# gplepage/lsqfit

Hardware: AMD Instinct MI355X
Metric: fp64 LM steps/sec at (N_data,N_param)=(65536,4096); chi2 match vs GSL (higher is better)
Workload: dtype f64

## Files before the change

lsqfit_amd/csrc/gemm_tn_f64.hip:

```cpp
#include <cstdlib>

#include "common.h"
#include <type_traits>
#include <vector>
#include "devmath.h"

namespace lsqamd {

#ifdef LSQAMD_SYRK_STAMPS
__device__ unsigned long long *g_syrk_stamps = nullptr;
#endif

typedef double v4d __attribute__((ext_vector_type(4)));
typedef double v2d __attribute__((ext_vector_type(2)));

constexpr int BM = 128, BN = 128, BK = 16;
constexpr int LDT = BM + 16;
constexpr int STAGE = 2 * BK * LDT;
constexpr size_t GEMM_LDS_BYTES = 2 * STAGE * sizeof(double);

struct GemmDev {
  const double *X, *Y;
  double *C;
  int64_t M, N, K, ldx, ldy, ldc;
// ... 22 lines not shown
  v.y = rowptr[i1];
  return v;
}

template <bool VEC>
__global__ __launch_bounds__(256, 2) void gemm_tn_f64_kernel(GemmDev g) {
  extern __shared__ __attribute__((aligned(16))) double smem[];
  const int tid = threadIdx.x;
  const int lane = tid & 63, wave = tid >> 6;
  const int wm = wave >> 1, wn = wave & 1;
  int tm, tn, split;
  if (g.work_map) {
    const int nw = g.n_work, bid = blockIdx.x;
    const int xcd = bid & 7, q = nw >> 3, r = nw & 7;
    const int w = (xcd < r ? xcd * (q + 1) : r * (q + 1) + (xcd - r) * q) + (bid >> 3);
    const int4 e = reinterpret_cast<const int4 *>(g.work_map)[w];
    tm = e.x; tn = e.y; split = e.z;
  } else {
    tm = blockIdx.x / g.tiles_n;
    tn = blockIdx.x % g.tiles_n;
    split = blockIdx.y;
  }
  const int64_t m0 = (int64_t)tm * BM, n0 = (int64_t)tn * BN;
  if (g.upper_only && n0 + BN <= m0) return;

  const int64_t b = blockIdx.z;
  if (g.batch_active && !g.batch_active[b]) return;
  const double *X = g.X + b * g.sx;
  const double *Y = g.Y + b * g.sy;
  double *C = g.C + b * g.sc + (int64_t)split * g.split_stride;

  int64_t kb = (int64_t)split * g.kchunk;
  int64_t ke = kb + g.kchunk < g.K ? kb + g.kchunk : g.K;
  if (g.x_upper_tri) {
    const int64_t lim = m0 + BM;
    if (ke > lim) ke = lim;
  }
  if (g.xy_lower_tri) {
    int64_t lo = m0 > n0 ? m0 : n0;
    lo -= lo % BK;
    if (kb < lo) kb = lo;
  }

  v4d acc[4][4];
#pragma unroll
  for (int i = 0; i < 4; ++i)
#pragma unroll
    for (int j = 0; j < 4; ++j) acc[i][j] = (v4d){0.0, 0.0, 0.0, 0.0};

  const int c2 = (tid & 63) * 2;
  const int rg = tid >> 6;
  const int64_t xc = m0 + c2, yc = n0 + c2;
  const bool x0ok = xc < g.M, x1ok = xc + 1 < g.M;
  const bool y0ok = yc < g.N, y1ok = yc + 1 < g.N;
  const int64_t xi0 = VEC ? (xc < g.ldx - 2 ? xc : g.ldx - 2) : (xc < g.M ? xc : g.M - 1);
  const int64_t xi1 = xc + 1 < g.M ? xc + 1 : g.M - 1;
  const int64_t yi0 = VEC ? (yc < g.ldy - 2 ? yc : g.ldy - 2) : (yc < g.N ? yc : g.N - 1);
  const int64_t yi1 = yc + 1 < g.N ? yc + 1 : g.N - 1;
  v2d xr[4], yr[4];

  auto gload = [&](int64_t k0) {
#pragma unroll
    for (int i = 0; i < 4; ++i) {
      int64_t row = k0 + rg + 4 * i;
      row = row < ke ? row : ke - 1;
      xr[i] = load2<VEC>(X + row * g.ldx, xi0, xi1);
      yr[i] = load2<VEC>(Y + row * g.ldy, yi0, yi1);
    }
  };
  auto sstore = [&](int buf, int64_t k0) {
    double *Xs = smem + buf * STAGE;
    double *Ys = Xs + BK * LDT;
#pragma unroll
    for (int i = 0; i < 4; ++i) {
      const int row = rg + 4 * i;
      const bool rok = k0 + row < ke;
      v2d xv, yv;
      xv.x = (rok && x0ok) ? xr[i].x : 0.0;
      xv.y = (rok && x1ok) ? xr[i].y : 0.0;
      yv.x = (rok && y0ok) ? yr[i].x : 0.0;
      yv.y = (rok && y1ok) ? yr[i].y : 0.0;
      *reinterpret_cast<v2d *>(Xs + row * LDT + c2) = xv;
      *reinterpret_cast<v2d *>(Ys + row * LDT + c2) = yv;
    }
  };

  const int fr = lane & 15, fq = lane >> 4;
  if (kb < ke) {
    gload(kb);
    sstore(0, kb);
  }
  __syncthreads();
  int cur = 0;
  for (int64_t k0 = kb; k0 < ke; k0 += BK) {
    const bool more = k0 + BK < ke;
    if (more) gload(k0 + BK);
    const double *Xs = smem + cur * STAGE;
    const double *Ys = Xs + BK * LDT;
#pragma unroll
    for (int kk = 0; kk < BK / 4; ++kk) {
      const int kr = kk * 4 + fq;
      double a[4], bb[4];
#pragma unroll
      for (int i = 0; i < 4; ++i) a[i] = Xs[kr * LDT + wm * 64 + i * 16 + fr];
#pragma unroll
      for (int j = 0; j < 4; ++j) bb[j] = Ys[kr * LDT + wn * 64 + j * 16 + fr];
#pragma unroll
      for (int i = 0; i < 4; ++i)
#pragma unroll
        for (int j = 0; j < 4; ++j)
          acc[i][j] = __builtin_amdgcn_mfma_f64_16x16x4f64(a[i], bb[j], acc[i][j], 0, 0, 0);
    }
    if (more) sstore(cur ^ 1, k0 + BK);
    __syncthreads();
    cur ^= 1;
  }

  const double alpha = g.alpha;
  const double beta = g.splits > 1 ? 0.0 : g.beta;
#pragma unroll
  for (int i = 0; i < 4; ++i) {
    double cv[4][4];
    if (beta != 0.0) {
#pragma unroll
      for (int j = 0; j < 4; ++j)
#pragma unroll
        for (int r = 0; r < 4; ++r) {
          const int64_t col = n0 + wn * 64 + j * 16 + fr;
          const int64_t row = m0 + wm * 64 + i * 16 + fq + 4 * r;
          const bool ok = col < g.N && row < g.M;
          cv[j][r] = C[(ok ? row : 0) * g.ldc + (ok ? col : 0)];
        }
    }
#pragma unroll
    for (int j = 0; j < 4; ++j) {
      const int64_t col = n0 + wn * 64 + j * 16 + fr;
      if (col >= g.N) continue;
#pragma unroll
      for (int r = 0; r < 4; ++r) {
        const int64_t row = m0 + wm * 64 + i * 16 + fq + 4 * r;
        if (row >= g.M) continue;
        double v = alpha * acc[i][j][r];
        if (beta != 0.0) v += beta * cv[j][r];
        C[row * g.ldc + col] = v;
      }
    }
  }
}

template <bool XTRI, bool WORKMAP, bool CS = false, bool SIGNAL = false>
__global__ __launch_bounds__(256, 2) void gemm_tn_f64_interior_kernel(GemmDev g) {
  extern __shared__ __attribute__((aligned(16))) double smem[];
  const int tid = threadIdx.x;
  const int lane = tid & 63, wave = tid >> 6;
  const int wm = wave >> 1, wn = wave & 1;
  int tm, tn, split;
  int sig_group = 0;
#ifdef LSQAMD_SYRK_STAMPS
  const unsigned long long stamp0 = __builtin_amdgcn_s_memrealtime();
  int stamp_w = -1;
#endif
  if (WORKMAP) {
    const int nw = g.n_work, bid = blockIdx.x;
    const int xcd = bid & 7, q = nw >> 3, r = nw & 7;
    const int w = (xcd < r ? xcd * (q + 1) : r * (q + 1) + (xcd - r) * q) + (bid >> 3);
#ifdef LSQAMD_SYRK_STAMPS
    stamp_w = w;
#endif
    const int4 e = reinterpret_cast<const int4 *>(g.work_map)[w];
    tm = e.x; tn = e.y; split = e.z;
    if (SIGNAL) sig_group = e.w;
  } else if (XTRI && g.xcd_groups) {
    const int L = blockIdx.x, xcd = L & 7, sl = L >> 3;
    const int gidx = xcd + 8 * (sl / g.tiles_n);
    tn = sl % g.tiles_n;
    tm = gidx % g.xcd_groups;
    split = gidx / g.xcd_groups;
  } else {
    tm = blockIdx.x / g.tiles_n;
    tn = blockIdx.x % g.tiles_n;
    split = blockIdx.y;
  }
  const int tm_other = (XTRI && g.pair_rows) ? g.tiles_m - 1 - tm : tm;
  const int npass = tm_other != tm ? 2 : 1;
  for (int pass = 0; pass < npass; ++pass) {
  if (pass >= 1) {
    tm = tm_other;
    __syncthreads();
  }
  const int64_t m0 = (int64_t)tm * BM, n0 = (int64_t)tn * BN;
  if (g.upper_only && n0 + BN <= m0) return;
  const int64_t b = blockIdx.z;
  if (g.batch_active && !g.batch_active[b]) return;
  double *C = g.C + b * g.sc + (int64_t)split * g.split_stride;
  int64_t kb = (int64_t)split * g.kchunk;
  int64_t ke = kb + g.kchunk < g.K ? kb + g.kchunk : g.K;
  if (g.x_upper_tri) {
    const int64_t lim = m0 + BM;
    if (ke > lim) ke = lim;
  }
  if (g.xy_lower_tri) {
    int64_t lo = m0 > n0 ? m0 : n0;
    lo -= lo % BK;
    if (kb < lo) kb = lo;
  }
  if (XTRI && g.tri_halves) {
    const int64_t lim = m0 + BM, h = (lim >> 1) & ~(int64_t)(BK - 1);
    kb = split ? h : 0;
    ke = split ? lim : h;
  }

  v4d acc[4][4];
#pragma unroll
  for (int i = 0; i < 4; ++i)
#pragma unroll
    for (int j = 0; j < 4; ++j) acc[i][j] = (v4d){0.0, 0.0, 0.0, 0.0};

  const bool diag = WORKMAP && !XTRI && g.syrk_diag && tm == tn;
  const int arow0 = diag ? (wave == 2 ? 32 : (wave == 3 ? 64 : 0)) : wm * 64;
  const int bcol0 = diag ? (wave == 0 ? 0 : 64) : wn * 64;

  typedef __attribute__((address_space(3))) void lds_void;
  typedef const __attribute__((address_space(1))) void glb_void;
  const double *xp = g.X + b * g.sx + (kb + wave) * g.ldx + m0 + 2 * lane;
  const double *yp = g.Y + b * g.sy + (kb + wave) * g.ldy + n0 + 2 * lane;
  const int64_t xstep = 4 * g.ldx, ystep = 4 * g.ldy;
  const char *fp = reinterpret_cast<const char *>(g.X + b * g.sx + (kb + (lane >> 1)) * g.ldx + g.colsum_rcol) + 4 * (lane & 1);
  const int64_t fstep = (int64_t)BK * g.ldx * (int64_t)sizeof(double);
  double cs = 0.0, cs2 = 0.0;

  auto stage = [&](int buf) {
    double *Xs = smem + buf * STAGE + wave * LDT;
    double *Ys = Xs + BK * LDT;
    if (diag) {
#pragma unroll
      for (int i = 0; i < 4; ++i)
        __builtin_amdgcn_global_load_lds((glb_void *)(xp + i * xstep), (lds_void *)(Xs + 4 * i * LDT), 16, 0, 0);
      if (CS && wave == 1) {
        if (lane < 32)
          __builtin_amdgcn_global_load_lds((glb_void *)fp, (lds_void *)(smem + buf * STAGE + BK * LDT), 4, 0, 0);
        fp += fstep;
      }
    } else {
#pragma unroll
      for (int i = 0; i < 4; ++i) {
        __builtin_amdgcn_global_load_lds((glb_void *)(xp + i * xstep), (lds_void *)(Xs + 4 * i * LDT), 16, 0, 0);
        __builtin_amdgcn_global_load_lds((glb_void *)(yp + i * ystep), (lds_void *)(Ys + 4 * i * LDT), 16, 0, 0);
      }
    }
    xp += 4 * xstep;
    yp += 4 * ystep;
  };

  const bool fuse = XTRI && g.colsum_out != nullptr;
  double wreg = 0.0;
  if (fuse && tid < BM) wreg = (g.C + b * g.sc)[(m0 + tid) * g.ldc + g.colsum_rcol];
  const int fr = lane & 15, fq = lane >> 4;
  if (kb < ke) stage(0);
  __syncthreads();
  auto kloop = [&](auto role_tag) {
    constexpr int ROLE = decltype(role_tag)::value;
    int cur = 0;
    for (int64_t k0 = kb; k0 < ke; k0 += BK) {
      if (k0 + BK < ke) stage(cur ^ 1);
      const double *Xs = smem + cur * STAGE;
      const double *Ys = ROLE == 0 ? Xs + BK * LDT : Xs;
#pragma unroll
      for (int kk = 0; kk < BK / 4; ++kk) {
        const int kr = kk * 4 + fq;
        double a[4], bb[4];
#pragma unroll
        for (int i = 0; i < (ROLE == 2 ? 2 : 4); ++i)
          a[i] = Xs[kr * LDT + (XTRI ? (2 * i + wm) * 16 : arow0 + i * 16) + fr];
#pragma unroll
        for (int j = 0; j < 4; ++j) bb[j] = Ys[kr * LDT + bcol0 + j * 16 + fr];
#pragma unroll
        for (int i = 0; i < (ROLE == 2 ? 2 : 4); ++i) {
          if (XTRI && k0 + kk * 4 > m0 + (2 * i + wm) * 16 + 15) continue;
#pragma unroll
          for (int j = (ROLE == 1 ? i : 0); j < 4; ++j)
            acc[i][j] = __builtin_amdgcn_mfma_f64_16x16x4f64(a[i], bb[j], acc[i][j], 0, 0, 0);
        }
      }
      if (CS && ROLE != 0) {
        const double *Fs = Xs + BK * LDT + 8 * (tid >> 7);
        const double *Xc = Xs + 8 * (tid >> 7) * LDT + (tid & 127);
#pragma unroll
        for (int r = 0; r < 8; ++r) {
          const double fv = Fs[r];
          cs = fma(Xc[r * LDT], fv, cs);
          cs2 = fma(fv, fv, cs2);
        }
      }
      __syncthreads();
      cur ^= 1;
    }
  };
  if (WORKMAP && !XTRI && diag) {
    if (wave == 0 || wave == 3) kloop(std::integral_constant<int, 1>{});
    else kloop(std::integral_constant<int, 2>{});
    const double alpha = g.alpha;
    const bool tri = wave == 0 || wave == 3;
#pragma unroll
    for (int i = 0; i < 4; ++i) {
      if (!tri && i >= 2) break;
#pragma unroll
      for (int j = 0; j < 4; ++j) {
        if (tri && j < i) continue;
        const int64_t col = n0 + bcol0 + j * 16 + fr;
#pragma unroll
        for (int r = 0; r < 4; ++r) {
          const int64_t row = m0 + arow0 + i * 16 + fq + 4 * r;
          const double v = alpha * acc[i][j][r];
          C[row * g.ldc + col] = v;
          if (!(tri && i == j)) C[col * g.ldc + row] = v;
        }
      }
    }
    if (CS) {
      smem[tid] = cs;
      if ((tid & 127) == 0) smem[256 + (tid >> 7)] = cs2;
      __syncthreads();
      double *out = g.colsum_out + (b * g.splits + split) * g.colsum_ld;
      if (tid < BM) out[m0 + tid] = smem[tid] + smem[tid + 128];
      if (tm == 0 && tid == 0) out[g.colsum_rcol] = smem[256] + smem[257];
    }
    continue;
  }
  kloop(std::integral_constant<int, 0>{});

  const double alpha = g.alpha;
  const double beta = g.splits > 1 ? 0.0 : g.beta;
  double *wcol = smem;
  double *red = smem + 128;
  if (fuse) {
    if (tid < BM) wcol[tid] = wreg;
    __syncthreads();
  }
  double sj[4] = {0.0, 0.0, 0.0, 0.0};
#pragma unroll
  for (int i = 0; i < 4; ++i) {
    const int rloc = (XTRI ? (2 * i + wm) * 16 : wm * 64 + i * 16) + fq;
    const int64_t rbase = m0 + rloc;
    double cv[4][4];
    if (beta != 0.0) {
#pragma unroll
      for (int j = 0; j < 4; ++j)
#pragma unroll
        for (int r = 0; r < 4; ++r)
          cv[j][r] = C[(rbase + 4 * r) * g.ldc + n0 + wn * 64 + j * 16 + fr];
    }
#pragma unroll
    for (int r = 0; r < 4; ++r) {
      const double w = fuse ? wcol[rloc + 4 * r] : 0.0;
#pragma unroll
      for (int j = 0; j < 4; ++j) {
        double v = alpha * acc[i][j][r];
        if (beta != 0.0) v += beta * cv[j][r];
        C[(rbase + 4 * r) * g.ldc + n0 + wn * 64 + j * 16 + fr] = v;
        if (XTRI) sj[j] += v * w;
      }
    }
  }
  if (fuse) {
#pragma unroll
    for (int j = 0; j < 4; ++j) {
      sj[j] += __shfl_xor(sj[j], 16, 64);
      sj[j] += __shfl_xor(sj[j], 32, 64);
    }
    if (fq == 0) {
#pragma unroll
      for (int j = 0; j < 4; ++j) red[wave * 64 + j * 16 + fr] = sj[j];
    }
    __syncthreads();
    if (wm == 0 && fq == 0) {
      double *out = g.colsum_out + (b * g.tiles_m + tm) * g.colsum_ld + n0 + wn * 64;
#pragma unroll
      for (int j = 0; j < 4; ++j) out[j * 16 + fr] = red[wave * 64 + j * 16 + fr] + red[(wave + 2) * 64 + j * 16 + fr];
    }
  }
  }
  if (SIGNAL && WORKMAP && sig_group > 0 && g.done_ctr) {
    asm volatile("s_waitcnt vmcnt(0)" ::: "memory");
    __syncthreads();
    if (tid == 0) {
      __builtin_amdgcn_fence(__ATOMIC_RELEASE, "agent");
      asm volatile("s_waitcnt vmcnt(0)" ::: "memory");
      __hip_atomic_fetch_add(g.done_ctr + (sig_group - 1), 1, __ATOMIC_RELAXED, __HIP_MEMORY_SCOPE_AGENT);
    }
  }
#ifdef LSQAMD_SYRK_STAMPS
  if (WORKMAP && g_syrk_stamps && tid == 0) {
    __builtin_amdgcn_s_waitcnt(0);
    unsigned long long *o = g_syrk_stamps + 5 * (size_t)blockIdx.x;
    o[0] = stamp0;
    o[1] = __builtin_amdgcn_s_memrealtime();
    o[2] = __builtin_amdgcn_s_getreg((3 << 11) | 20);
    o[3] = __builtin_amdgcn_s_getreg((31 << 11) | 4);
    o[4] = (unsigned long long)stamp_w;
  }
#endif
}

constexpr int TS = 64;
constexpr int LDS_S = TS + 16;
constexpr int STAGE_S = 2 * BK * LDS_S;
constexpr size_t GEMM_LDS_BYTES_S = 2 * STAGE_S * sizeof(double);

template <bool VEC>
__global__ __launch_bounds__(256, 4) void gemm_tn_f64_small_kernel(GemmDev g) {
  extern __shared__ __attribute__((aligned(16))) double smem[];
  const int tid = threadIdx.x;
  const int lane = tid & 63, wave = tid >> 6;
  const int wm = wave >> 1, wn = wave & 1;
  const int tm = blockIdx.x / g.tiles_n, tn = blockIdx.x % g.tiles_n;
  const int split = blockIdx.y;
  const int64_t m0 = (int64_t)tm * TS, n0 = (int64_t)tn * TS;
  if (g.upper_only && n0 + TS <= m0) return;
  const int64_t b = blockIdx.z;
  if (g.batch_active && !g.batch_active[b]) return;
  const double *X = g.X + b * g.sx;
  const double *Y = g.Y + b * g.sy;
  double *C = g.C + b * g.sc + (int64_t)split * g.split_stride;
  int64_t kb = (int64_t)split * g.kchunk;
  int64_t ke = kb + g.kchunk < g.K ? kb + g.kchunk : g.K;
  if (g.x_upper_tri) {
    const int64_t lim = m0 + TS;
    if (ke > lim) ke = lim;
  }
  if (g.xy_lower_tri) {
    int64_t lo = m0 > n0 ? m0 : n0;
    lo -= lo % BK;
    if (kb < lo) kb = lo;
  }
  v4d acc[2][2];
#pragma unroll
  for (int i = 0; i < 2; ++i)
#pragma unroll
    for (int j = 0; j < 2; ++j) acc[i][j] = (v4d){0.0, 0.0, 0.0, 0.0};

  const int c2 = (tid & 31) * 2;
  const int rg = tid >> 5;
  const int64_t xc = m0 + c2, yc = n0 + c2;
  const bool x0ok = xc < g.M, x1ok = xc + 1 < g.M;
  const bool y0ok = yc < g.N, y1ok = yc + 1 < g.N;
  const int64_t xi0 = VEC ? (xc < g.ldx - 2 ? xc : g.ldx - 2) : (xc < g.M ? xc : g.M - 1);
  const int64_t xi1 = xc + 1 < g.M ? xc + 1 : g.M - 1;
  const int64_t yi0 = VEC ? (yc < g.ldy - 2 ? yc : g.ldy - 2) : (yc < g.N ? yc : g.N - 1);
// ... 427 lines not shown
      }
    }
    hipLaunchKernelGGL((gemm_tn_f64_interior_kernel<true, false>), grid, dim3(256), GEMM_LDS_BYTES, st, g);
  }
  else if (interior && a.work_map && a.colsum_out) {
    if (!g.syrk_diag || !a.upper_only) return hipErrorInvalidValue;
    if (g.done_ctr) hipLaunchKernelGGL((gemm_tn_f64_interior_kernel<false, true, true, true>), grid, dim3(256), GEMM_LDS_BYTES, st, g);
    else hipLaunchKernelGGL((gemm_tn_f64_interior_kernel<false, true, true>), grid, dim3(256), GEMM_LDS_BYTES, st, g);
  }
  else if (interior && a.work_map && g.done_ctr)
    hipLaunchKernelGGL((gemm_tn_f64_interior_kernel<false, true, false, true>), grid, dim3(256), GEMM_LDS_BYTES, st, g);
  else if (interior && a.work_map)
    hipLaunchKernelGGL((gemm_tn_f64_interior_kernel<false, true>), grid, dim3(256), GEMM_LDS_BYTES, st, g);
  else if (interior)
    hipLaunchKernelGGL((gemm_tn_f64_interior_kernel<false, false>), grid, dim3(256), GEMM_LDS_BYTES, st, g);
  else if (g.vec_x && g.vec_y)
    hipLaunchKernelGGL(gemm_tn_f64_kernel<true>, grid, dim3(256), GEMM_LDS_BYTES, st, g);
  else
    hipLaunchKernelGGL(gemm_tn_f64_kernel<false>, grid, dim3(256), GEMM_LDS_BYTES, st, g);
  return hipGetLastError();
}

int64_t syrk_work_count(int64_t P, int32_t splits) {
  const int64_t T = (P + BM - 1) / BM;
  return T * (T + 1) / 2 * (splits < 1 ? 1 : splits);
}

void syrk_work_fill(int64_t P, int32_t splits, int32_t *out) { (void)syrk_work_fill_rows(P, splits, 0, (int)((P + BM - 1) / BM), out); }

int64_t syrk_work_fill_rows(int64_t P, int32_t splits, int row0, int row1, int32_t *out) {
  const int T = (int)((P + BM - 1) / BM), PS = 8;
  const int NP = (T + PS - 1) / PS;
  if (row0 < 0) row0 = 0;
  if (row1 > T) row1 = T;
  int64_t o = 0;
  for (int s = 0; s < (splits < 1 ? 1 : splits); ++s)
    for (int pi = 0; pi < NP; ++pi)
      for (int pj = pi; pj < NP; ++pj)
        for (int tm = pi * PS; tm < (pi + 1) * PS && tm < T; ++tm) {
          if (tm < row0 || tm >= row1) continue;
          for (int tn = pj * PS; tn < (pj + 1) * PS && tn < T; ++tn) {
            if (tn < tm) continue;
            out[o++] = tm; out[o++] = tn; out[o++] = s; out[o++] = 0;
          }
        }
  const int64_t nw = o / 4, q = nw / 8, r = nw % 8;
  std::vector<int32_t> tmp;
  for (int xcd = 0; xcd < 8; ++xcd) {
    const int64_t b = xcd < r ? xcd * (q + 1) : r * (q + 1) + (xcd - r) * q, n = q + (xcd < r ? 1 : 0);
    tmp.assign(out + 4 * b, out + 4 * (b + n));
    int64_t w = b;
    for (int keep = 0; keep < 2; ++keep)
      for (int64_t e = 0; e < n; ++e)
        if ((tmp[4 * e] == tmp[4 * e + 1]) == (keep == 1)) {
          for (int c = 0; c < 4; ++c) out[4 * w + c] = tmp[4 * e + c];
          ++w;
        }
  }
  return nw;
}

void syrk_work_fill_grouped(int64_t P, int32_t splits, int G, const int32_t *rows, int32_t *out, int32_t *count) {
  const int64_t nw = syrk_work_count(P, splits), q = nw / 8, r = nw % 8;
  std::vector<std::vector<int32_t>> lists((size_t)G);
  for (int g = 0; g < G; ++g) {
    lists[(size_t)g].resize(4 * (size_t)nw);
    const int T = (int)((P + BM - 1) / BM), PS = 8, NP = (T + PS - 1) / PS;
    int64_t o = 0;
    int32_t *L = lists[(size_t)g].data();
    for (int s = 0; s < (splits < 1 ? 1 : splits); ++s)
      for (int pi = 0; pi < NP; ++pi)
        for (int pj = pi; pj < NP; ++pj)
          for (int tm = pi * PS; tm < (pi + 1) * PS && tm < T; ++tm) {
            if (tm < rows[g] || tm >= rows[g + 1]) continue;
            for (int tn = pj * PS; tn < (pj + 1) * PS && tn < T; ++tn) {
              if (tn < tm) continue;
              L[o++] = tm; L[o++] = tn; L[o++] = s; L[o++] = g + 1;
            }
          }
    lists[(size_t)g].resize((size_t)o);
    count[g] = (int32_t)(o / 4);
  }
  std::vector<int64_t> cap(8), pos((size_t)G, 0);
  for (int x = 0; x < 8; ++x) cap[(size_t)x] = q + (x < r ? 1 : 0);
  std::vector<std::vector<int64_t>> c((size_t)G, std::vector<int64_t>(8, 0));
  for (int g = 0; g < G; ++g) {
    if (g == G - 1) {
      for (int x = 0; x < 8; ++x) c[(size_t)g][(size_t)x] = cap[(size_t)x];
      break;
    }
    int64_t left = count[g];
    for (int x = 0; x < 8; ++x) {
      int64_t v = count[g] / 8;
      if (v > cap[(size_t)x]) v = cap[(size_t)x];
      c[(size_t)g][(size_t)x] = v;
      cap[(size_t)x] -= v;
      left -= v;
    }
    while (left > 0) {
      int best = 0;
      for (int x = 1; x < 8; ++x)
        if (cap[(size_t)x] > cap[(size_t)best]) best = x;
      c[(size_t)g][(size_t)best]++;
      cap[(size_t)best]--;
      --left;
    }
  }
  int64_t w = 0;
  for (int x = 0; x < 8; ++x)
    for (int g = 0; g < G; ++g) {
      const int32_t *L = lists[(size_t)g].data() + 4 * pos[(size_t)g];
      const int64_t n = c[(size_t)g][(size_t)x];
      for (int keep = 0; keep < 2; ++keep)
        for (int64_t e = 0; e < n; ++e)
          if ((L[4 * e] == L[4 * e + 1]) == (keep == 1)) {
            for (int k = 0; k < 4; ++k) out[4 * w + k] = L[4 * e + k];
            ++w;
          }
      pos[(size_t)g] += n;
    }
}

__global__ __launch_bounds__(64) void wait_counter_kernel(const int32_t *ctr, int32_t expect, int32_t *timed_out) {
  if (threadIdx.x != 0) return;
  const unsigned long long t0 = __builtin_amdgcn_s_memrealtime();
  while (__hip_atomic_load(ctr, __ATOMIC_RELAXED, __HIP_MEMORY_SCOPE_AGENT) < expect) {
    __builtin_amdgcn_s_sleep(64);
    if (__builtin_amdgcn_s_memrealtime() - t0 > 400000000ull) {
      __hip_atomic_store(timed_out, 1, __ATOMIC_RELAXED, __HIP_MEMORY_SCOPE_AGENT);
      break;
    }
  }
}

hipError_t launch_wait_counter(hipStream_t st, const int32_t *ctr, int32_t expect, int32_t *timed_out) {
  hipLaunchKernelGGL(wait_counter_kernel, dim3(1), dim3(64), 0, st, ctr, expect, timed_out);
  return hipGetLastError();
}

template <int MODEL, int NT, bool FAR>
__global__ __launch_bounds__(256, 2) void whiten_synth_kernel(WhitenSynth a, int tiles_m, int tiles_n, int pair_rows) {
  extern __shared__ __attribute__((aligned(16))) double smem[];
  if (a.trig_far && (a.trig_far[0] != 0) != FAR) return;
  const int tid = threadIdx.x;
  const int lane = tid & 63, wave = __builtin_amdgcn_readfirstlane(tid >> 6);
  const int wm = wave >> 1, wn = wave & 1;
  const int tm_first = blockIdx.x / tiles_n, tn = blockIdx.x % tiles_n;
  const int npass = (pair_rows && tiles_m - 1 - tm_first != tm_first) ? 2 : 1;
  for (int pass = 0; pass < npass; ++pass) {
  if (pass == 1) __syncthreads();
  const int tm = pass == 0 ? tm_first : tiles_m - 1 - tm_first;
  const int64_t b = blockIdx.z;
  const int64_t m0 = (int64_t)tm * BM;
  const int64_t ke = m0 + BM;
  const double *Xb = a.Wt + b * a.B * a.B;
  const double *xrow = a.x + b * a.B;
  double *C = a.J + b * a.B * a.ld;
  constexpr int NJ = NT / 16;
  constexpr int SR = 256 / NT, NS = BK / SR;
  const int sc = tid % NT, srow = tid / NT;
  const double amp = a.p[(int64_t)tn * NT + sc], frq = a.p[a.K + (int64_t)tn * NT + sc];

  v4d acc[4][NJ];
#pragma unroll
  for (int i = 0; i < 4; ++i)
#pragma unroll
    for (int j = 0; j < NJ; ++j) acc[i][j] = (v4d){0.0, 0.0, 0.0, 0.0};
  typedef __attribute__((address_space(3))) void lds_void;
  typedef const __attribute__((address_space(1))) void glb_void;
  const double *xp = Xb + (int64_t)wave * a.B + m0 + 2 * lane;
  const int64_t xstep = 4 * a.B;
  double *xring = smem + 2 * STAGE;
  auto xdma = [&](int64_t sidx) {
    if (wave == 0) {
      int64_t e = sidx * BK + (lane >> 1);
      if (e > a.B - 1) e = a.B - 1;
      const char *src = reinterpret_cast<const char *>(xrow + e) + 4 * (lane & 1);
      __builtin_amdgcn_global_load_lds((glb_void *)src, (lds_void *)(xring + (sidx % 3) * 32), 4, 0, 0);
    }
  };
  int64_t ssyn = 0;
  auto stage_dma = [&](int buf) {
    double *Xs = smem + buf * STAGE + wave * LDT;
#pragma unroll
    for (int i = 0; i < 4; ++i)
      __builtin_amdgcn_global_load_lds((glb_void *)(xp + i * xstep), (lds_void *)(Xs + 4 * i * LDT), 16, 0, 0);
    xp += 4 * xstep;
  };
  auto stage_synth = [&](int buf) {
    double xs4[NS];
    const double *xq = xring + (ssyn % 3) * 32 + srow;
#pragma unroll
    for (int i = 0; i < NS; ++i) xs4[i] = xq[SR * i];
    double *Ys = smem + buf * STAGE + BK * LDT;
#pragma unroll
    for (int i = 0; i < NS; ++i) {
      const int row = srow + SR * i;
      const double xv = xs4[i];
      double t, dq;
      if (MODEL == LSQAMD_MODEL_COSMIX) {
        double sn, cs;
        sincos_moderate<FAR>(frq * xv, &sn, &cs);
        t = cs;
        dq = -amp * xv * sn;
      } else {
        const double e = exp(-frq * xv);
        t = e;
        dq = -amp * xv * e;
      }
      Ys[row * LDT + sc] = t;
      Ys[row * LDT + NT + sc] = dq;
    }
    ++ssyn;
  };
  const double wreg = (tid < BM) ? C[(m0 + tid) * a.ld + 2 * a.K] : 0.0;
  const int fr = lane & 15, fq = lane >> 4;
  xdma(0);
  xdma(1);
  stage_dma(0);
  __syncthreads();
  stage_synth(0);
  __syncthreads();
  int cur = 0;
  for (int64_t k0 = 0; k0 < ke; k0 += BK) {
    if (k0 + BK < ke) {
      if (k0 + 2 * BK < ke) xdma(k0 / BK + 2);
      stage_dma(cur ^ 1);
      stage_synth(cur ^ 1);
    }
    const double *Xs = smem + cur * STAGE;
    const double *Ys = Xs + BK * LDT;
#pragma unroll
    for (int kk = 0; kk < BK / 4; ++kk) {
      const int kr = kk * 4 + fq;
      double av[4], bb[NJ];
#pragma unroll
      for (int i = 0; i < 4; ++i) av[i] = Xs[kr * LDT + (2 * i + wm) * 16 + fr];
#pragma unroll
      for (int j = 0; j < NJ; ++j) bb[j] = Ys[kr * LDT + wn * NT + j * 16 + fr];
#pragma unroll
      for (int i = 0; i < 4; ++i) {
        if (k0 + kk * 4 > m0 + (2 * i + wm) * 16 + 15) continue;
#pragma unroll
        for (int j = 0; j < NJ; ++j)
          acc[i][j] = __builtin_amdgcn_mfma_f64_16x16x4f64(av[i], bb[j], acc[i][j], 0, 0, 0);
      }
    }
    __syncthreads();
    cur ^= 1;
  }
  double *wcol = smem, *red = smem + 128;
  if (tid < BM) wcol[tid] = wreg;
  __syncthreads();
  const int64_t cbase = (wn ? a.K : 0) + (int64_t)tn * NT;
  double sj[NJ];
#pragma unroll
  for (int j = 0; j < NJ; ++j) sj[j] = 0.0;
#pragma unroll
  for (int i = 0; i < 4; ++i) {
    const int rloc = (2 * i + wm) * 16 + fq;
#pragma unroll
    for (int r = 0; r < 4; ++r) {
      const double w = wcol[rloc + 4 * r];
#pragma unroll
      for (int j = 0; j < NJ; ++j) {
        const double v = acc[i][j][r];
        C[(m0 + rloc + 4 * r) * a.ld + cbase + j * 16 + fr] = v;
        sj[j] += v * w;
      }
    }
  }
#pragma unroll
  for (int j = 0; j < NJ; ++j) {
    sj[j] += __shfl_xor(sj[j], 16, 64);
    sj[j] += __shfl_xor(sj[j], 32, 64);
  }
  if (fq == 0) {
#pragma unroll
    for (int j = 0; j < NJ; ++j) red[wave * 64 + j * 16 + fr] = sj[j];
  }
  __syncthreads();
  if (wm == 0 && fq == 0) {
    double *out = a.colsum_out + (b * tiles_m + tm) * (2 * a.K) + cbase;
#pragma unroll
    for (int j = 0; j < NJ; ++j) out[j * 16 + fr] = red[wave * 64 + j * 16 + fr] + red[(wave + 2) * 64 + j * 16 + fr];
  }
  }
}


bool whiten_synth_eligible(int32_t model, int64_t B, int64_t P) {
  const char *e = getenv("LSQAMD_FUSED_JACOBIAN");
  const bool off = e && e[0] == '0', always = e && e[0] == '2';
  return !off && (model == LSQAMD_MODEL_COSMIX || model == LSQAMD_MODEL_MULTIEXP) && B >= BM && B % BM == 0 &&
         (B < 8 * BM || always) && P % 128 == 0 && P >= 128;
}

constexpr size_t SYNTH_LDS_BYTES = GEMM_LDS_BYTES + 3 * 32 * sizeof(double);

template <int MODEL, int NT, bool FAR>
static hipError_t launch_whiten_synth_one(hipStream_t st, const WhitenSynth &a, dim3 grid, int tiles_m, int tiles_n, int pair) {
  static PerDeviceOnce attr;
  const hipError_t ea = attr.run([] {
    return hipFuncSetAttribute(reinterpret_cast<const void *>(whiten_synth_kernel<MODEL, NT, FAR>),
                               hipFuncAttributeMaxDynamicSharedMemorySize, (int)SYNTH_LDS_BYTES);
  });
  if (ea != hipSuccess) return ea;
  hipLaunchKernelGGL((whiten_synth_kernel<MODEL, NT, FAR>), grid, dim3(256), SYNTH_LDS_BYTES, st, a, tiles_m, tiles_n, pair);
  return hipGetLastError();
}

template <int MODEL, int NT>
static hipError_t launch_whiten_synth_nt(hipStream_t st, const WhitenSynth &a, dim3 grid, int tiles_m, int tiles_n, int pair) {
  if (MODEL == LSQAMD_MODEL_COSMIX && a.trig_far) {
    hipError_t e = launch_whiten_synth_one<MODEL, NT, false>(st, a, grid, tiles_m, tiles_n, pair);
    if (e != hipSuccess) return e;
  }
  return launch_whiten_synth_one<MODEL, NT, true>(st, a, grid, tiles_m, tiles_n, pair);
}

hipError_t launch_whiten_synth(hipStream_t st, const WhitenSynth &a0) {
  WhitenSynth a = a0;
  if (a.model != LSQAMD_MODEL_COSMIX) a.trig_far = nullptr;
  const int tiles_m = (int)(a.B / BM);
  const int pair = tiles_m >= 4 ? 1 : 0;
  const int64_t rows = pair ? (tiles_m + 1) / 2 : tiles_m;
  static const int64_t narrow_below = [] { const char *e = getenv("LSQAMD_SYNTH_NARROW"); return e ? atoll(e) : (int64_t)400; }();
  const bool narrow = rows * (a.K / 64) * a.nb < narrow_below && a.K % 32 == 0;
  const int tiles_n = (int)(a.K / (narrow ? 32 : 64));
  dim3 grid((unsigned)(rows * tiles_n), 1, (unsigned)a.nb);
  if (a.model == LSQAMD_MODEL_COSMIX)
    return narrow ? launch_whiten_synth_nt<LSQAMD_MODEL_COSMIX, 32>(st, a, grid, tiles_m, tiles_n, pair)
                  : launch_whiten_synth_nt<LSQAMD_MODEL_COSMIX, 64>(st, a, grid, tiles_m, tiles_n, pair);
  return narrow ? launch_whiten_synth_nt<LSQAMD_MODEL_MULTIEXP, 32>(st, a, grid, tiles_m, tiles_n, pair)
                : launch_whiten_synth_nt<LSQAMD_MODEL_MULTIEXP, 64>(st, a, grid, tiles_m, tiles_n, pair);
}

}

#ifdef LSQAMD_SYRK_STAMPS
extern "C" int lsqamd_debug_set_syrk_stamps(void *dev_ptr) try {
  return (int)hipMemcpyToSymbol(HIP_SYMBOL(lsqamd::g_syrk_stamps), &dev_ptr, sizeof(void *));
} LSQAMD_ABI_CATCH(return lsqamd::abi_exception(nullptr);)
#endif
```

Before: 50.03.

## Split k-loop into full and triangular phases with compile-time buffer indices

Restructures the GEMM-TN interior and whiten-synth k-loops. Each loop is unrolled by two with constexpr double-buffer indices, and full stages are separated from the diagonal triangular stages, so the per-MFMA triangle check disappears from the bulk of the loop. Wave and work-map indices are made scalar with readfirstlane, and LDS pointers and a lane offset are precomputed to cut VALU address arithmetic. The cost is more code and higher register pressure, and the new stage counting adds risk of off-by-one errors at tile boundaries.

```diff
diff --git a/lsqfit_amd/csrc/gemm_tn_f64.hip b/lsqfit_amd/csrc/gemm_tn_f64.hip
--- a/lsqfit_amd/csrc/gemm_tn_f64.hip
+++ b/lsqfit_amd/csrc/gemm_tn_f64.hip
@@ -198,7 +198,7 @@
 __global__ __launch_bounds__(256, 2) void gemm_tn_f64_interior_kernel(GemmDev g) {
   extern __shared__ __attribute__((aligned(16))) double smem[];
   const int tid = threadIdx.x;
-  const int lane = tid & 63, wave = tid >> 6;
+  const int lane = tid & 63, wave = __builtin_amdgcn_readfirstlane(tid >> 6);
   const int wm = wave >> 1, wn = wave & 1;
   int tm, tn, split;
   int sig_group = 0;
@@ -214,8 +214,10 @@
     stamp_w = w;
 #endif
     const int4 e = reinterpret_cast<const int4 *>(g.work_map)[w];
-    tm = e.x; tn = e.y; split = e.z;
-    if (SIGNAL) sig_group = e.w;
+    tm = __builtin_amdgcn_readfirstlane(e.x);
+    tn = __builtin_amdgcn_readfirstlane(e.y);
+    split = __builtin_amdgcn_readfirstlane(e.z);
+    if (SIGNAL) sig_group = __builtin_amdgcn_readfirstlane(e.w);
   } else if (XTRI && g.xcd_groups) {
     const int L = blockIdx.x, xcd = L & 7, sl = L >> 3;
     const int gidx = xcd + 8 * (sl / g.tiles_n);
@@ -268,20 +270,24 @@
 
   typedef __attribute__((address_space(3))) void lds_void;
   typedef const __attribute__((address_space(1))) void glb_void;
-  const double *xp = g.X + b * g.sx + (kb + wave) * g.ldx + m0 + 2 * lane;
-  const double *yp = g.Y + b * g.sy + (kb + wave) * g.ldy + n0 + 2 * lane;
-  const int64_t xstep = 4 * g.ldx, ystep = 4 * g.ldy;
+  const char *xb = reinterpret_cast<const char *>(g.X + b * g.sx + (kb + wave) * g.ldx + m0);
+  const char *yb = reinterpret_cast<const char *>(g.Y + b * g.sy + (kb + wave) * g.ldy + n0);
+  const int64_t xstep = 4 * g.ldx * (int64_t)sizeof(double), ystep = 4 * g.ldy * (int64_t)sizeof(double);
+  uint32_t lane_off = 16u * (uint32_t)lane;
+  const int nst = kb < ke ? (int)((ke - kb + BK - 1) >> 4) : 0;
   const char *fp = reinterpret_cast<const char *>(g.X + b * g.sx + (kb + (lane >> 1)) * g.ldx + g.colsum_rcol) + 4 * (lane & 1);
   const int64_t fstep = (int64_t)BK * g.ldx * (int64_t)sizeof(double);
   double cs = 0.0, cs2 = 0.0;
 
-  auto stage = [&](int buf) {
+  auto stage = [&](auto buf_tag) {
+    constexpr int buf = decltype(buf_tag)::value;
+    asm volatile("" : "+v"(lane_off));
     double *Xs = smem + buf * STAGE + wave * LDT;
     double *Ys = Xs + BK * LDT;
     if (diag) {
 #pragma unroll
       for (int i = 0; i < 4; ++i)
-        __builtin_amdgcn_global_load_lds((glb_void *)(xp + i * xstep), (lds_void *)(Xs + 4 * i * LDT), 16, 0, 0);
+        __builtin_amdgcn_global_load_lds((glb_void *)(xb + i * xstep + lane_off), (lds_void *)(Xs + 4 * i * LDT), 16, 0, 0);
       if (CS && wave == 1) {
         if (lane < 32)
           __builtin_amdgcn_global_load_lds((glb_void *)fp, (lds_void *)(smem + buf * STAGE + BK * LDT), 4, 0, 0);
@@ -290,42 +296,69 @@
     } else {
 #pragma unroll
       for (int i = 0; i < 4; ++i) {
-        __builtin_amdgcn_global_load_lds((glb_void *)(xp + i * xstep), (lds_void *)(Xs + 4 * i * LDT), 16, 0, 0);
-        __builtin_amdgcn_global_load_lds((glb_void *)(yp + i * ystep), (lds_void *)(Ys + 4 * i * LDT), 16, 0, 0);
-      }
-    }
-    xp += 4 * xstep;
-    yp += 4 * ystep;
+        __builtin_amdgcn_global_load_lds((glb_void *)(xb + i * xstep + lane_off), (lds_void *)(Xs + 4 * i * LDT), 16, 0, 0);
+        __builtin_amdgcn_global_load_lds((glb_void *)(yb + i * ystep + lane_off), (lds_void *)(Ys + 4 * i * LDT), 16, 0, 0);
+      }
+    }
+    xb += 4 * xstep;
+    yb += 4 * ystep;
   };
 
   const bool fuse = XTRI && g.colsum_out != nullptr;
   double wreg = 0.0;
   if (fuse && tid < BM) wreg = (g.C + b * g.sc)[(m0 + tid) * g.ldc + g.colsum_rcol];
   const int fr = lane & 15, fq = lane >> 4;
-  if (kb < ke) stage(0);
+  if (nst > 0) stage(std::integral_constant<int, 0>{});
   __syncthreads();
   auto kloop = [&](auto role_tag) {
     constexpr int ROLE = decltype(role_tag)::value;
-    int cur = 0;
-    for (int64_t k0 = kb; k0 < ke; k0 += BK) {
-      if (k0 + BK < ke) stage(cur ^ 1);
+    typedef const __attribute__((address_space(3))) double lds_cdouble;
+    lds_cdouble *ap[2][BK / 4], *bp[2][BK / 4];
+#pragma unroll
+    for (int c = 0; c < 2; ++c)
+#pragma unroll
+      for (int kk = 0; kk < BK / 4; ++kk) {
+        const double *Xk = smem + c * STAGE + (kk * 4 + fq) * LDT + fr;
+        ap[c][kk] = (lds_cdouble *)(Xk + (XTRI ? wm * 16 : arow0));
+        bp[c][kk] = (lds_cdouble *)(Xk + (ROLE == 0 ? BK * LDT : 0) + bcol0);
+        asm volatile("" : "+v"(ap[c][kk]), "+v"(bp[c][kk]));
+      }
+    auto body = [&](auto cur_tag, auto tri_tag, const int ts, const bool more) {
+      constexpr int cur = decltype(cur_tag)::value;
+      constexpr bool TRI = XTRI && decltype(tri_tag)::value != 0;
+      if (more) stage(std::integral_constant<int, cur ^ 1>{});
       const double *Xs = smem + cur * STAGE;
-      const double *Ys = ROLE == 0 ? Xs + BK * LDT : Xs;
-#pragma unroll
-      for (int kk = 0; kk < BK / 4; ++kk) {
-        const int kr = kk * 4 + fq;
-        double a[4], bb[4];
-#pragma unroll
-        for (int i = 0; i < (ROLE == 2 ? 2 : 4); ++i)
-          a[i] = Xs[kr * LDT + (XTRI ? (2 * i + wm) * 16 : arow0 + i * 16) + fr];
-#pragma unroll
-        for (int j = 0; j < 4; ++j) bb[j] = Ys[kr * LDT + bcol0 + j * 16 + fr];
-#pragma unroll
-        for (int i = 0; i < (ROLE == 2 ? 2 : 4); ++i) {
-          if (XTRI && k0 + kk * 4 > m0 + (2 * i + wm) * 16 + 15) continue;
-#pragma unroll
-          for (int j = (ROLE == 1 ? i : 0); j < 4; ++j)
-            acc[i][j] = __builtin_amdgcn_mfma_f64_16x16x4f64(a[i], bb[j], acc[i][j], 0, 0, 0);
+      if (TRI) {
+        double bb[BK / 4][4];
+#pragma unroll
+        for (int kk = 0; kk < BK / 4; ++kk)
+#pragma unroll
+          for (int j = 0; j < 4; ++j) bb[kk][j] = bp[cur][kk][j * 16];
+#pragma unroll
+        for (int i = 0; i < 4; ++i) {
+          if (2 * i + wm < ts) continue;
+          double a[BK / 4];
+#pragma unroll
+          for (int kk = 0; kk < BK / 4; ++kk) a[kk] = ap[cur][kk][2 * i * 16];
+#pragma unroll
+          for (int kk = 0; kk < BK / 4; ++kk)
+#pragma unroll
+            for (int j = 0; j < 4; ++j)
+              acc[i][j] = __builtin_amdgcn_mfma_f64_16x16x4f64(a[kk], bb[kk][j], acc[i][j], 0, 0, 0);
+        }
+      } else {
+#pragma unroll
+        for (int kk = 0; kk < BK / 4; ++kk) {
+          double a[4], bb[4];
+#pragma unroll
+          for (int i = 0; i < (ROLE == 2 ? 2 : 4); ++i) a[i] = ap[cur][kk][(XTRI ? 2 * i : i) * 16];
+#pragma unroll
+          for (int j = 0; j < 4; ++j) bb[j] = bp[cur][kk][j * 16];
+#pragma unroll
+          for (int i = 0; i < (ROLE == 2 ? 2 : 4); ++i)
+#pragma unroll
+            for (int j = (ROLE == 1 ? i : 0); j < 4; ++j)
+              acc[i][j] = __builtin_amdgcn_mfma_f64_16x16x4f64(a[i], bb[j], acc[i][j], 0, 0, 0);
         }
       }
       if (CS && ROLE != 0) {
@@ -339,7 +372,32 @@
         }
       }
       __syncthreads();
-      cur ^= 1;
+    };
+    using c0_tag = std::integral_constant<int, 0>;
+    using c1_tag = std::integral_constant<int, 1>;
+    int nfull = nst;
+    if (XTRI) {
+      const int64_t below = kb < m0 ? (m0 - kb) >> 4 : 0;
+      nfull = below < nst ? (int)below : nst;
+    }
+    int s = 0;
+    for (; s + 1 < nfull; s += 2) {
+      body(c0_tag{}, c0_tag{}, 0, true);
+      body(c1_tag{}, c0_tag{}, 0, s + 2 < nst);
+    }
+    if (s < nfull) body(c0_tag{}, c0_tag{}, 0, s + 1 < nst);
+    if (XTRI && nfull < nst) {
+      const int t1 = (int)((kb + (int64_t)nst * BK - m0) >> 4);
+      int t = t1 - (nst - nfull);
+      if (nfull & 1) {
+        body(c1_tag{}, c1_tag{}, t, t + 1 < t1);
+        ++t;
+      }
+      for (; t + 1 < t1; t += 2) {
+        body(c0_tag{}, c1_tag{}, t, true);
+        body(c1_tag{}, c1_tag{}, t + 1, t + 2 < t1);
+      }
+      if (t < t1) body(c0_tag{}, c1_tag{}, t, false);
     }
   };
   if (WORKMAP && !XTRI && diag) {
@@ -1073,7 +1131,6 @@
   const int tm = pass == 0 ? tm_first : tiles_m - 1 - tm_first;
   const int64_t b = blockIdx.z;
   const int64_t m0 = (int64_t)tm * BM;
-  const int64_t ke = m0 + BM;
   const double *Xb = a.Wt + b * a.B * a.B;
   const double *xrow = a.x + b * a.B;
   double *C = a.J + b * a.B * a.ld;
@@ -1089,26 +1146,30 @@
     for (int j = 0; j < NJ; ++j) acc[i][j] = (v4d){0.0, 0.0, 0.0, 0.0};
   typedef __attribute__((address_space(3))) void lds_void;
   typedef const __attribute__((address_space(1))) void glb_void;
-  const double *xp = Xb + (int64_t)wave * a.B + m0 + 2 * lane;
-  const int64_t xstep = 4 * a.B;
+  const char *xb = reinterpret_cast<const char *>(Xb + (int64_t)wave * a.B + m0);
+  const int64_t xstep = 4 * a.B * (int64_t)sizeof(double);
+  uint32_t lane_off = 16u * (uint32_t)lane;
   double *xring = smem + 2 * STAGE;
-  auto xdma = [&](int64_t sidx) {
+  auto xdma = [&](int sidx) {
     if (wave == 0) {
-      int64_t e = sidx * BK + (lane >> 1);
+      int64_t e = (int64_t)sidx * BK + (lane >> 1);
       if (e > a.B - 1) e = a.B - 1;
       const char *src = reinterpret_cast<const char *>(xrow + e) + 4 * (lane & 1);
       __builtin_amdgcn_global_load_lds((glb_void *)src, (lds_void *)(xring + (sidx % 3) * 32), 4, 0, 0);
     }
   };
-  int64_t ssyn = 0;
-  auto stage_dma = [&](int buf) {
+  int ssyn = 0;
+  auto stage_dma = [&](auto buf_tag) {
+    constexpr int buf = decltype(buf_tag)::value;
+    asm volatile("" : "+v"(lane_off));
     double *Xs = smem + buf * STAGE + wave * LDT;
 #pragma unroll
     for (int i = 0; i < 4; ++i)
-      __builtin_amdgcn_global_load_lds((glb_void *)(xp + i * xstep), (lds_void *)(Xs + 4 * i * LDT), 16, 0, 0);
-    xp += 4 * xstep;
+      __builtin_amdgcn_global_load_lds((glb_void *)(xb + i * xstep + lane_off), (lds_void *)(Xs + 4 * i * LDT), 16, 0, 0);
+    xb += 4 * xstep;
   };
-  auto stage_synth = [&](int buf) {
+  auto stage_synth = [&](auto buf_tag) {
+    constexpr int buf = decltype(buf_tag)::value;
     double xs4[NS];
     const double *xq = xring + (ssyn % 3) * 32 + srow;
 #pragma unroll
@@ -1136,19 +1197,25 @@
   };
   const double wreg = (tid < BM) ? C[(m0 + tid) * a.ld + 2 * a.K] : 0.0;
   const int fr = lane & 15, fq = lane >> 4;
+  using c0_tag = std::integral_constant<int, 0>;
+  using c1_tag = std::integral_constant<int, 1>;
   xdma(0);
   xdma(1);
-  stage_dma(0);
+  stage_dma(c0_tag{});
   __syncthreads();
-  stage_synth(0);
+  stage_synth(c0_tag{});
   __syncthreads();
-  int cur = 0;
-  for (int64_t k0 = 0; k0 < ke; k0 += BK) {
-    if (k0 + BK < ke) {
-      if (k0 + 2 * BK < ke) xdma(k0 / BK + 2);
-      stage_dma(cur ^ 1);
-      stage_synth(cur ^ 1);
-    }
+  const int nst = 8 * (tm + 1);
+  auto next = [&](auto cur_tag, const int sidx) {
+    constexpr int cur = decltype(cur_tag)::value;
+    if (sidx + 1 < nst) {
+      if (sidx + 2 < nst) xdma(sidx + 2);
+      stage_dma(std::integral_constant<int, cur ^ 1>{});
+      stage_synth(std::integral_constant<int, cur ^ 1>{});
+    }
+  };
+  auto mfmas_full = [&](auto cur_tag) {
+    constexpr int cur = decltype(cur_tag)::value;
     const double *Xs = smem + cur * STAGE;
     const double *Ys = Xs + BK * LDT;
 #pragma unroll
@@ -1160,15 +1227,50 @@
 #pragma unroll
       for (int j = 0; j < NJ; ++j) bb[j] = Ys[kr * LDT + wn * NT + j * 16 + fr];
 #pragma unroll
-      for (int i = 0; i < 4; ++i) {
-        if (k0 + kk * 4 > m0 + (2 * i + wm) * 16 + 15) continue;
+      for (int i = 0; i < 4; ++i)
 #pragma unroll
         for (int j = 0; j < NJ; ++j)
           acc[i][j] = __builtin_amdgcn_mfma_f64_16x16x4f64(av[i], bb[j], acc[i][j], 0, 0, 0);
-      }
-    }
+    }
+  };
+  auto mfmas_tri = [&](auto cur_tag, const int ts) {
+    constexpr int cur = decltype(cur_tag)::value;
+    const double *Xs = smem + cur * STAGE;
+    const double *Ys = Xs + BK * LDT;
+    double bb[BK / 4][NJ];
+#pragma unroll
+    for (int kk = 0; kk < BK / 4; ++kk)
+#pragma unroll
+      for (int j = 0; j < NJ; ++j) bb[kk][j] = Ys[(kk * 4 + fq) * LDT + wn * NT + j * 16 + fr];
+#pragma unroll
+    for (int i = 0; i < 4; ++i) {
+      if (2 * i + wm < ts) continue;
+      double av[BK / 4];
+#pragma unroll
+      for (int kk = 0; kk < BK / 4; ++kk) av[kk] = Xs[(kk * 4 + fq) * LDT + (2 * i + wm) * 16 + fr];
+#pragma unroll
+      for (int kk = 0; kk < BK / 4; ++kk)
+#pragma unroll
+        for (int j = 0; j < NJ; ++j)
+          acc[i][j] = __builtin_amdgcn_mfma_f64_16x16x4f64(av[kk], bb[kk][j], acc[i][j], 0, 0, 0);
+    }
+  };
+  const int nfull = 8 * tm;
+  for (int s = 0; s < nfull; s += 2) {
+    next(c0_tag{}, s);
+    mfmas_full(c0_tag{});
     __syncthreads();
-    cur ^= 1;
+    next(c1_tag{}, s + 1);
+    mfmas_full(c1_tag{});
+    __syncthreads();
+  }
+  for (int t = 0; t < 8; t += 2) {
+    next(c0_tag{}, nfull + t);
+    mfmas_tri(c0_tag{}, t);
+    __syncthreads();
+    next(c1_tag{}, nfull + t + 1);
+    mfmas_tri(c1_tag{}, t + 1);
+    __syncthreads();
   }
   double *wcol = smem, *red = smem + 128;
   if (tid < BM) wcol[tid] = wreg;
```

Result: faster. 54.10 (median of 6 runs) (+8.1%).
